# neka-nat/cupoch

Hardware: AMD Instinct MI355X
Metric: ICP iterations/sec (incl. kNN) on 10M-pt point-to-plane, 1/2/4/8 MI355X (higher is better)
Workload: dtype f32; 1 GPU; 10M-vs-10M point-to-plane ICP, radius 1-NN on an 8-ary kd-cell tree, r=2*N^(-1/3), uniform random clouds (BASELINE.md section 3); points=10000000, parallelism=single GPU, accumulate=f64

## Files before the change

cupoch_amd/_lib.py:

```python
import ctypes as C
import os
import shutil
import subprocess

_HERE = os.path.dirname(os.path.abspath(__file__))
ROOT = os.path.dirname(_HERE)
CSRC = os.path.join(_HERE, "csrc")
LIB_DIR = os.path.join(_HERE, "lib")
LIB_PATH = os.path.join(LIB_DIR, "libmi_icp.so")
INCLUDE = os.path.join(ROOT, "include")

HIPCC_FLAGS = ["--offload-arch=gfx950", "-O3", "-std=c++17", "-ffp-contract=off", "-fPIC", "-I/opt/rocm/include"]
UNITS = ["mi_icp", "mi_build", "mi_geometry", "mi_knn", "mi_comm", "mi_debug"]
OBJ_DIR = os.path.join(LIB_DIR, "obj")

MI_ICP_HOST, MI_ICP_DEVICE = 0, 1
EST_POINT_TO_POINT, EST_POINT_TO_PLANE, EST_SYMMETRIC, EST_GENERALIZED = 1, 2, 3, 5
EST_COLORED = 4


class MiIcpError(RuntimeError):
    pass


# ... 136 lines not shown
    "mi_icp_estimate_normals_knn": (_I, [_P, _P, _L, _I, _P, _I]),
    "mi_icp_estimate_normals_radius": (_I, [_P, _P, _L, _F, _I, _P, _I]),
    "mi_icp_search_knn": (_I, [_P, _P, _L, _I, _F, _P, _P, C.POINTER(_L), _I]),
    "mi_icp_set_target_colors": (_I, [_P, _P, _I]),
    "mi_icp_set_source_colors": (_I, [_P, _P, _I]),
    "mi_icp_set_lambda_geometric": (_I, [_P, _F]),
    "mi_icp_compute_color_gradients": (_I, [_P, _F, _I, _P, _I]),
    "mi_icp_registration_colored_icp": (_I, [_P, _F, _P, C.POINTER(Params), _F, C.POINTER(Result)]),
    "mi_icp_comm_unique_id": (_I, [_P]),
    "mi_icp_comm_init": (_I, [_P, _P, _I, _I]),
    "mi_icp_comm_init_local": (_I, [_P, C.c_char_p, _I, _I]),
    "mi_icp_comm_kind": (_I, [_P]),
    "mi_icp_comm_autotune": (_I, [_P, _I, _P, _P]),
    "mi_icp_comm_destroy": (_I, [_P]),
    "mi_icp_set_global_source_count": (_I, [_P, _L]),
    "mi_icp_spatial_order": (_I, [_P, _P, _L, _P, _I]),
    "mi_icp_set_iteration_callback": (_I, [_P, _P, _P]),
    "mi_icp_set_profiling": (_I, [_P, _I]),
    "mi_icp_get_profile": (_I, [_P, _P]),
    "mi_icp_debug_sort_pairs": (_I, [_P, _P, _P, _L, _I]),
    "mi_icp_debug_exclusive_scan": (_I, [_P, _P, _P, _L, _P]),
    "mi_icp_debug_morton_order": (_I, [_P, _P, _L, _P]),
    "mi_icp_debug_nn_stats": (_I, [_P, _P, _F, _I, _P]),
    "mi_icp_debug_nn_stats8": (_I, [_P, _P, _F, _I, _P]),
    "mi_icp_debug_get_tree": (_I, [_P, C.POINTER(_L), _P, _P]),
    "mi_icp_debug_drop_seeds": (_I, [_P]),
    "mi_icp_debug_last_search_kind": (_I, [_P]),
    "mi_icp_debug_last_voxel_path": (_I, [_P]),
    "mi_icp_debug_occupancy": (_I, [_I]),
    "mi_icp_debug_loop_counters": (_I, [_P, _P]),
    "mi_icp_debug_search_skip": (_I, [_P, _P, _P, _L, C.POINTER(_L), C.POINTER(_I)]),
    "mi_icp_debug_locate": (_I, [_P, _P, _P]),
    "mi_icp_debug_set_step_stamps": (_I, [_P, _I]),
    "mi_icp_debug_get_step_stamps": (_I, [_P, _P, C.POINTER(C.c_double)]),
    "mi_icp_debug_solve_both": (_I, [_I, _P, _I, C.c_float, _P, _P, _P, _P]),
    "mi_icp_debug_get_leaf_regions": (_I, [_P, _P]),
    "mi_icp_debug_get_leaf_halos": (_I, [_P, _P]),
    "mi_icp_debug_eigen3": (_I, [_I, _P, _L, _P, _P, _P]),
    "mi_icp_debug_odometry_image": (_I, [_P, _I, _I, _P, C.POINTER(_I), C.POINTER(_I)]),
}

_lib = None


def load():
    global _lib
    if _lib is not None:
        return _lib
    override = os.environ.get("MI_ICP_LIB_PATH")
    path = override or LIB_PATH
    if not os.path.exists(path):
        raise MiIcpError(
            "libmi_icp.so is not built (%s). Run `python -c 'import __graft_entry__ as g; "
            "g.build()'` or cupoch_amd._lib.build(); there is no CPU fallback." % LIB_PATH)
    try:
        lib = C.CDLL(path, mode=C.RTLD_GLOBAL)
    except OSError as e:
        raise MiIcpError("cannot load %s: %s" % (path, e))
    for name, (res, args) in SIGNATURES.items():
        if override and name.startswith("mi_icp_debug_") and not hasattr(lib, name):
            continue
        fn = getattr(lib, name)
        fn.restype = res
        fn.argtypes = args
    _lib = lib
    return lib
# ... 1 lines not shown
```

cupoch_amd/csrc/ctx.h:

```cpp
#pragma once
#include <hip/hip_runtime.h>
#include <rccl/rccl.h>

#include <algorithm>
#include <cmath>
#include <cstdarg>
#include <cstdio>
#include <cstdlib>
#include <cstring>
#include <string>

#include "../../include/mi_icp.h"
#include "../../include/mi_icp_debug.h"
#include "device_utils.h"
#include "host_solver.h"
#include "loop.h"
#include "mailbox.h"
#include "primitives.h"

namespace mi {
namespace eng {

using host::Mat4;

// ... 56 lines not shown

    mi::eng::DevBuf user_pairs;
    int64_t n_user_pairs = -1;

    mi::eng::DevBuf keys0, keys1, vals0, vals1, hist, scan_tmp, bounds_part, bounds;
    mi::eng::DevBuf partial, sys_dev, dense_idx, flags, pairs_out, seg_start;
    mi::eng::DevBuf stage[6];
    mi::eng::DevBuf tscale;
    mi::eng::DevBuf knn_idx, knn_flags;
    mi::eng::DevBuf dbs[4];
    mi::eng::DevBuf seg[4];
    float vx_refused_voxel = 0.0f;
    int64_t vx_refused_n = 0;
    int vx_order = 0;
    mi::eng::DevBuf vx_tab;
    mi::eng::DevBuf vpay[6];
    double* sys_host = nullptr;
    float* f_host = nullptr;
    uint32_t* u_host = nullptr;
    void* od_host = nullptr;
    int od_levels = 0, od_lw[MI_ICP_ODOMETRY_MAX_LEVELS] = {}, od_lh[MI_ICP_ODOMETRY_MAX_LEVELS] = {};
    const float* od_img[MI_ICP_ODOMETRY_MAX_LEVELS][8] = {};

    mi::eng::DevBuf loop_dev, ticket;
    mi::DevLoop* loop_host = nullptr;
    bool loop_active = false;
    mi_icp_iteration_fn iter_fn = nullptr;
    void* iter_user = nullptr;
    mi::eng::DevBuf loop_hist;
    float* hist_host = nullptr;
    int iter_reported = 0;
    float loop_r2 = 0.0f;
    int loop_est = 0;

    ncclComm_t comm = nullptr;
    int nranks = 1, rank = 0;
    mi::MailBox* mail_host = nullptr;
    mi::MailBox* mail_dev = nullptr;
    size_t mail_bytes = 0;
    std::string mail_name;
    bool mail_linked = false;
    unsigned long long* inbox = nullptr;
    unsigned long long* inbox_peer[mi::kMailRanks] = {};
    mi::eng::DevBuf inbox_table;
    bool comm_broken = false;
    int xchg = 0;
    uint32_t tune_epoch = 0;
    mi::eng::DevBuf mail_state;

    mi_icp_ctx* aux = nullptr;

    mi::eng::DevBuf stamps;
    bool stamps_on = false;
    bool profiling = false;
    static constexpr int kEvPairs = 16;
    hipEvent_t ev[4] = {nullptr, nullptr, nullptr, nullptr};
    hipEvent_t evp[2][kEvPairs][2] = {};
    int evp_n[2] = {0, 0};
    bool ev_pending_nn = false, ev_pending_red = false;
    double prof[8] = {0, 0, 0, 0, 0, 0, 0, 0};
};

namespace mi {
namespace eng {

inline float* lreg_of(const mi_icp_ctx* c) { return c->tblk.p ? (float*)c->tblk.p + mi::kLeafRegOffset : nullptr; }
// ... 72 lines not shown
        return MI_ICP_OK;
    }
    return ensure(c, stage, count, out);
}

template <class T>
int from_device(mi_icp_ctx* c, const T* dev, T* dst, size_t count, int mem_kind) {
    if (!dst || dst == dev || count == 0) return MI_ICP_OK;
    HIPCHK(c, hipMemcpyAsync(dst, dev, count * sizeof(T),
                             mem_kind == MI_ICP_DEVICE ? hipMemcpyDeviceToDevice
                                                       : hipMemcpyDeviceToHost,
                             c->stream));
    return MI_ICP_OK;
}

inline int drop_expiry(mi_icp_ctx* c) {
    c->skip_r2 = NAN;
    if (c->expiry_live && c->expiry.p) HIPCHK(c, hipMemsetAsync(c->expiry.p, 0xff, c->expiry.bytes, c->stream));
    c->expiry_live = false;
    return MI_ICP_OK;
}

inline uint32_t skip_live_shift(int64_t ns) {
    uint32_t shift = 0;
    while ((((ns + 63) / 64) >> (shift + 1)) >= 64) ++shift;
    return shift;
}
inline bool skip_pays(const mi_icp_ctx* c) {
    if (!c->loop_host || c->ns <= 0) return false;
    const int64_t samples = std::min<int64_t>(64, ((c->ns + 63) / 64) >> skip_live_shift(c->ns));
    int64_t held = 0;
    for (int64_t k = 0; k < samples; ++k) held += c->loop_host->live[k] ? 1 : 0;
    return samples > 0 && held * 4 >= samples;
}

inline int blocks_for(int64_t n, int per = 256) { return (int)std::max<int64_t>(1, (n + per - 1) / per); }

inline Xform make_xform(const Mat4& T) { return xform_from(T); }

inline Mat4 load_T(const float* T) {
    if (!T) return host::identity4();
    Mat4 m;
    std::memcpy(m.data(), T, sizeof(float) * 16);
    return m;
}

struct EvTimer {
    mi_icp_ctx* c;
    int slot;
    hipEvent_t stop = nullptr;
    bool pooled;
    EvTimer(mi_icp_ctx* ctx, int s, bool in_loop) : c(ctx), slot(s), pooled(in_loop) {
        if (!c->profiling) return;
        if (pooled) {
            if (c->evp_n[slot] >= mi_icp_ctx::kEvPairs) return;
            const int i = c->evp_n[slot]++;
            (void)hipEventRecord(c->evp[slot][i][0], c->stream);
            stop = c->evp[slot][i][1];
        } else {
            (void)hipEventRecord(c->ev[slot * 2], c->stream);
            stop = c->ev[slot * 2 + 1];
        }
    }
    ~EvTimer() {
        if (!stop) return;
        (void)hipEventRecord(stop, c->stream);
// ... 87 lines not shown
```

cupoch_amd/csrc/mi_debug.hip:

```cpp
#include "ctx.h"
#include <vector>
#include "halo_format.h"
#include "traverse.h"
#include "wave_solver.h"
#include "eigen3.h"

using namespace mi;
using namespace mi::eng;
using host::Mat4;

namespace mi {
__global__ __launch_bounds__(64) void solve_both_kernel(const double* systems, float det_thresh, float* out_serial,
                                                        float* out_wave, int32_t* ok_serial, int32_t* ok_wave) {
    __shared__ double s_sys[32];
    const int n = (int)blockIdx.x;
    if (threadIdx.x < 32) s_sys[threadIdx.x] = systems[(int64_t)n * 32 + threadIdx.x];
    __syncthreads();
    host::Mat4 W;
    const bool okw = wave_solve_system(s_sys, det_thresh, W);
    if (threadIdx.x < 16) out_wave[(int64_t)n * 16 + threadIdx.x] = select16(W.m, (int)threadIdx.x);
    if (threadIdx.x == 0) {
        ok_wave[n] = okw ? 1 : 0;
        host::Mat4 S;
        ok_serial[n] = host::solve_system(s_sys, det_thresh, S) ? 1 : 0;
// ... 116 lines not shown

int mi_icp_debug_solve_both(int device, const double* systems, int n, float det_thresh, float* out_serial,
                            float* out_wave, int32_t* ok_serial, int32_t* ok_wave) {
    if (!systems || n <= 0 || !out_serial || !out_wave || !ok_serial || !ok_wave) return MI_ICP_ERR_INVALID;
    if (hipSetDevice(device) != hipSuccess) return MI_ICP_ERR_NO_DEVICE;
    double* d_sys = nullptr;
    float* d_out = nullptr;
    int32_t* d_ok = nullptr;
    int rc = MI_ICP_ERR_HIP;
    if (hipMalloc(&d_sys, (size_t)n * 32 * sizeof(double)) == hipSuccess &&
        hipMalloc(&d_out, (size_t)n * 32 * sizeof(float)) == hipSuccess &&
        hipMalloc(&d_ok, (size_t)n * 2 * sizeof(int32_t)) == hipSuccess &&
        hipMemcpy(d_sys, systems, (size_t)n * 32 * sizeof(double), hipMemcpyHostToDevice) == hipSuccess) {
        mi::solve_both_kernel<<<n, 64>>>(d_sys, det_thresh, d_out, d_out + (size_t)n * 16, d_ok, d_ok + n);
        if (hipDeviceSynchronize() == hipSuccess &&
            hipMemcpy(out_serial, d_out, (size_t)n * 16 * sizeof(float), hipMemcpyDeviceToHost) == hipSuccess &&
            hipMemcpy(out_wave, d_out + (size_t)n * 16, (size_t)n * 16 * sizeof(float), hipMemcpyDeviceToHost) == hipSuccess &&
            hipMemcpy(ok_serial, d_ok, (size_t)n * sizeof(int32_t), hipMemcpyDeviceToHost) == hipSuccess &&
            hipMemcpy(ok_wave, d_ok + n, (size_t)n * sizeof(int32_t), hipMemcpyDeviceToHost) == hipSuccess)
            rc = MI_ICP_OK;
    }
    (void)hipFree(d_sys);
    (void)hipFree(d_out);
    (void)hipFree(d_ok);
    return rc;
}

int mi_icp_debug_set_step_stamps(mi_icp_ctx* c, int enable) {
    TRY(check_ctx(c));
    c->stamps_on = enable != 0;
    return MI_ICP_OK;
}

int mi_icp_debug_get_step_stamps(mi_icp_ctx* c, uint64_t* out32, double* ticks_per_us) {
    TRY(check_ctx(c));
    if (!out32 || !c->stamps.p) return fail(c, MI_ICP_ERR_STATE, "debug_get_step_stamps: no stamped loop has run on this context");
    HIPCHK(c, hipStreamSynchronize(c->stream));
    HIPCHK(c, hipMemcpy(out32, c->stamps.p, sizeof(uint64_t) * kStampWords, hipMemcpyDeviceToHost));
    if (ticks_per_us) {
        int khz = 0;
        *ticks_per_us = (hipDeviceGetAttribute(&khz, hipDeviceAttributeWallClockRate, c->device) == hipSuccess && khz > 0) ? khz / 1000.0 : 100.0;
    }
    return MI_ICP_OK;
}

int mi_icp_debug_loop_counters(mi_icp_ctx* c, int32_t* out4) {
    TRY(check_ctx(c));
    if (!out4 || !c->loop_host) return fail(c, MI_ICP_ERR_INVALID, "debug_loop_counters: bad arguments");
    HIPCHK(c, hipStreamSynchronize(c->stream));
    out4[0] = c->loop_host->iterations;
    out4[1] = c->loop_host->passes;
    out4[2] = c->loop_host->relocations;
    out4[3] = c->relocate_armed ? 1 : 0;
    return MI_ICP_OK;
}

int mi_icp_debug_drop_seeds(mi_icp_ctx* c) {
    TRY(check_ctx(c));
    c->nn_valid = false;
    return drop_expiry(c);
}

int mi_icp_debug_search_skip(mi_icp_ctx* c, double* state2, double* limits_out, int64_t capacity, int64_t* npackets, int* armed) {
    TRY(check_ctx(c));
    if (!state2 || !npackets || !armed || capacity < 0) return fail(c, MI_ICP_ERR_INVALID, "debug_search_skip: bad arguments");
    if (!c->loop_active || !c->loop_dev.p || !c->expiry.p || c->ns <= 0)
// ... 94 lines not shown
```

cupoch_amd/csrc/mi_icp.hip:

```cpp
#include "ctx.h"
#include "fused_small.h"
#include "lzf.h"
#include "nn_search.h"
#include "reduce.h"

using namespace mi;
using namespace mi::eng;
using host::Mat4;

namespace mi {

static __global__ __launch_bounds__(kStepThreads) void loop_step_kernel(DevLoop* st_g, double* sys_in, int resume, MailArgs mail) {
    __shared__ DevLoop st_s;
    loop_step_block(st_g, sys_in, resume, st_s, StepPre{false, 0u, 0.0, 0u}, mail);
}

namespace eng {

constexpr int64_t kPt2PlTwoFrom = (int64_t)4 << 20;

static int64_t coarse_first_min() {
    static const int64_t v = [] { const char* s = std::getenv("MI_ICP_COARSE_MIN"); return s ? std::atoll(s) : (int64_t)1 << 16; }();
    return v;
}
// ... 35 lines not shown
static decltype(&nn_packet_kernel<false, false>) nn_kernel(bool seeded, bool stats, bool stamp, bool gate) {
    if (gate) return stamp ? nn_packet_kernel<true, false, true, true> : nn_packet_kernel<true, false, false, true>;
    if (stats) return seeded ? nn_packet_kernel<true, true> : nn_packet_kernel<false, true>;
    if (seeded && stamp) return nn_packet_kernel<true, false, true>;
    return seeded ? nn_packet_kernel<true, false> : nn_packet_kernel<false, false>;
}

int launch_nn(mi_icp_ctx* c, const Mat4& T, float r2, bool seed, unsigned long long* stats, const DevLoop* loop) {
    if (c->ns <= 0) return MI_ICP_OK;
    int32_t* idx = (int32_t*)c->nn_idx.p;
    if (c->nt <= 0) {
        TRY(drop_expiry(c));
        fill_i32<<<blocks_for(c->ns), 256, 0, c->stream>>>(idx, c->ns, -1);
        KCHK(c);
        c->nn_valid = true;
        c->n_user_pairs = -1;
        return MI_ICP_OK;
    }
    const Xform X = make_xform(T);
    const bool use_seed = seed && c->nn_valid;
    bool have_halo;
    uint32_t* want = nullptr;
    if (loop) {
        TRY(loop_halo(c, &have_halo, &want));
    } else {
        if (use_seed) TRY(ensure_links(c));
        have_halo = halo_poll(c);
    }
    EvTimer t(c, 0, loop != nullptr);
    const bool self_seeded = !use_seed && !stats && c->ns >= coarse_first_min() && have_halo && planes_available(c);
    const bool limits = loop != nullptr && (use_seed || self_seeded) && !stats && c->expiry.p != nullptr;
    const bool may_skip = limits && use_seed && c->expiry_live && c->skip_r2 == r2;
    if (!may_skip) TRY(drop_expiry(c));
    const uint32_t run = (may_skip && skip_pays(c)) ? kSkipRun : 1u;
    if (self_seeded) TRY(launch_locate_by_planes(c, X, loop, 0));
    c->last_search_kind = use_seed ? 1 : (self_seeded ? 2 : 0);
    const PacketGrid g = packet_grid(c->ns, run);
    nn_kernel(use_seed || self_seeded, stats != nullptr, loop && c->stamps_on, run > 1u)<<<g.grid, kNNThreads, 0, c->stream>>>(
            (const float*)c->sx.p, (const float*)c->sy.p, (const float*)c->sz.p, (int)c->ns, (const float*)c->nodes.p,
            (const float*)c->tblk.p, (const float*)lreg_of(c), have_halo ? (const float*)c->thalo.p : nullptr, c->leaf_first,
            X, loop, r2, g.nblocks, idx, loop ? nullptr : (float*)c->nn_d2.p, stats, want,
            limits ? (double*)c->expiry.p : nullptr,
            limits ? reinterpret_cast<uint8_t*>(c->loop_dev.p) + offsetof(DevLoop, live) : nullptr, skip_live_shift(c->ns), run);
    KCHK(c);
    if (limits) {
        c->expiry_live = true;
        c->skip_r2 = r2;
    }
    c->nn_valid = true;
    c->n_user_pairs = -1;
    return MI_ICP_OK;
}

int occupancy_loop(int which) {
    int blocks = -1;
    hipError_t e = hipErrorInvalidValue;
    if (which == 1) e = hipOccupancyMaxActiveBlocksPerMultiprocessor(&blocks, nn_packet_kernel<true, false>, kNNThreads, 0);
    else if (which == 2) e = hipOccupancyMaxActiveBlocksPerMultiprocessor(&blocks, nn_packet_kernel<false, false>, kNNThreads, 0);
    else if (which == 3) e = hipOccupancyMaxActiveBlocksPerMultiprocessor(&blocks, reduce_pt2pl_kernel<2, 1>, kReduceThreads, 0);
    else return -1;
    return e == hipSuccess ? blocks : -2;
}

}
}

namespace {

int ensure_inverse_maps(mi_icp_ctx* c) {
    if (!c->inv_s_valid && c->ns > 0) {
        int32_t* inv;
        TRY(ensure(c, c->inv_s, (size_t)c->ns, &inv));
        invert_perm_source<<<blocks_for(c->ns), 256, 0, c->stream>>>((const int32_t*)c->sperm.p, (int)c->ns, inv);
        KCHK(c);
        c->inv_s_valid = true;
    }
// ... 56 lines not shown
        case kEstP2P: return reduce_kernel<kEstP2P, MODE>;
        case kEstPt2Pl: return reduce_kernel<kEstPt2Pl, MODE>;
        case kEstSym: return reduce_kernel<kEstSym, MODE>;
        case kEstColored: return reduce_kernel<kEstColored, MODE>;
        case kEstGICP: return reduce_kernel<kEstGICP, MODE>;
        default: return nullptr;
    }
}

int launch_reduce(mi_icp_ctx* c, int est, int mode, const Mat4& T, DevLoop* loop = nullptr, int step = 0) {
    double *partial, *sys;
    uint32_t* ticket;
    TRY(reduce_buffers(c, kReduceBlocks, &partial, &sys, &ticket));
    ReduceArgs a;
    a.sx = (const float*)c->sx.p;
    a.sy = (const float*)c->sy.p;
    a.sz = (const float*)c->sz.p;
    a.snrm = (const float4*)c->snrm.p;
    a.scov = (const float*)c->scov.p;
    a.tblk = (const float*)c->tblk.p;
    a.tnrm = (const float4*)c->tnrm.p;
    a.trec = c->t_has_rec ? (const float*)c->trec.p : nullptr;
    a.tcov = (const float*)c->tcov.p;
    a.tgrad = (const float4*)c->tgrad.p;
    a.sint = (const float*)c->sint.p;
    a.sqrt_lambda_geometric = std::sqrt(c->lambda_geometric);
    a.sqrt_lambda_photometric = std::sqrt(1.0f - c->lambda_geometric);
    a.nn_idx = (const int32_t*)c->nn_idx.p;
    a.pairs = nullptr;
    a.inv_s = a.inv_t = nullptr;
    a.ns = (int)c->ns;
    a.nt = (int)c->nt;
    a.count = c->ns;
    if (c->n_user_pairs >= 0) {
        TRY(ensure_inverse_maps(c));
        a.pairs = (const int32_t*)c->user_pairs.p;
        a.inv_s = (const int32_t*)c->inv_s.p;
        a.inv_t = (const int32_t*)c->inv_t.p;
        a.count = c->n_user_pairs;
    }
    if (c->ns <= 0 || c->nt <= 0 || (!a.pairs && !c->nn_valid)) a.count = 0;
    const int64_t wide = std::min<int64_t>(256, blocks_for(a.count, kReduceThreads));
    const int grid = (int)std::max<int64_t>(
            wide, std::min<int64_t>(kReduceBlocks, blocks_for(a.count, kReduceThreads * kReduceElemsPerThread)));
    const Xform X = make_xform(T);
    if (pt2pl_reduction(c, est, mode)) {
        const auto kernel = (a.count >= kPt2PlTwoFrom) ? pt2pl_kernel<2>(step, c->stamps_on) : pt2pl_kernel<4>(step, c->stamps_on);
        EvTimer t(c, 1, loop != nullptr);
        kernel<<<std::min(grid, 512), kReduceThreads, 0, c->stream>>>(a, X, loop, partial, ticket, sys,
                                                                     (step == 2) ? mail_args(c) : MailArgs{});
        KCHK(c);
        return MI_ICP_OK;
    }
    if (!estimator_ready(c, est)) {
        est = kEstP2P;
        mode = 1;
    }
    const auto kernel = mode ? generic_reduce_kernel<1>(est) : generic_reduce_kernel<0>(est);
    if (!kernel) return fail(c, MI_ICP_ERR_INVALID, "unknown estimation type %d", est);
    EvTimer t(c, 1, loop != nullptr);
    kernel<<<grid, kReduceThreads, 0, c->stream>>>(a, X, loop, partial, ticket, sys);
    KCHK(c);
    return MI_ICP_OK;
}

int fetch_system(mi_icp_ctx* c, double* out) {
    double* sys = (double*)c->sys_dev.p;
    TRY(allreduce_system(c));
    HIPCHK(c, hipMemcpyAsync(c->sys_host, sys, kSysSize * sizeof(double), hipMemcpyDeviceToHost, c->stream));
    const bool mail = mail_on(c);
    int32_t* err_host = reinterpret_cast<int32_t*>(c->sys_host + 40);
    if (mail) HIPCHK(c, hipMemcpyAsync(err_host, (const int32_t*)c->mail_state.p + 1, sizeof(int32_t), hipMemcpyDeviceToHost, c->stream));
    HIPCHK(c, hipStreamSynchronize(c->stream));
    collect_events(c);
    if (mail && *err_host) return comm_failed(c, "the ranks' exchange timed out (mailbox): a peer did not post its sums");
    std::memcpy(out, c->sys_host, kSysSize * sizeof(double));
    return MI_ICP_OK;
}

Mat4 solve_update(const mi_icp_ctx* c, int est, const double* sys, float det_thresh) {
// ... 371 lines not shown
    TRY(drop_expiry(c));
    const PacketGrid g = packet_grid(c->ns, kFusedPackets);
    double *partial, *sys;
    uint32_t* ticket;
    TRY(reduce_buffers(c, std::max<uint32_t>(kReduceBlocks, g.grid), &partial, &sys, &ticket));
    EvTimer t(c, 0, true);
    const auto kernel = (c->loop_est == kEstP2P) ? icp_small_iteration_kernel<kEstP2P> : icp_small_iteration_kernel<kEstPt2Pl>;
    kernel<<<g.grid, kReduceThreads, 0, c->stream>>>(
            (const float*)c->sx.p, (const float*)c->sy.p, (const float*)c->sz.p, (int)c->ns, (const float*)c->nodes.p,
            (const float*)c->tblk.p, (const float*)lreg_of(c), have_halo ? (const float*)c->thalo.p : nullptr, c->leaf_first,
            c->loop_r2, g.npackets, g.nblocks, (int32_t*)c->nn_idx.p, want, (const float*)c->trec.p, d, partial, ticket, sys);
    KCHK(c);
    c->last_search_kind = 1;
    return MI_ICP_OK;
}

static int step_in_reduction(const mi_icp_ctx* c) {
    if (!pt2pl_reduction(c, c->loop_est, 0)) return 0;
    if (mail_on(c)) return 2;
    return (!c->comm && !c->mail_dev) ? 1 : 0;
}

static int loop_enqueue_evaluation(mi_icp_ctx* c, bool seed) {
    DevLoop* d = (DevLoop*)c->loop_dev.p;
    if (seed && c->relocate_armed && c->halo_use && c->nn_valid && c->n_user_pairs < 0 && c->ns > 0 && c->nt > 0) {
        const Xform none = {};
        TRY(launch_locate_by_planes(c, none, d, 1));
    }
    if (fused_iteration_applies(c, seed)) return launch_fused_iteration(c, d);
    const Mat4 I = host::identity4();
    TRY(launch_nn(c, I, c->loop_r2, seed, nullptr, d));
    const int step = step_in_reduction(c);
    TRY(launch_reduce(c, c->loop_est, 0, I, d, step));
    if (step) return MI_ICP_OK;
    const bool mail = mail_on(c);
    if (!mail) TRY(allreduce_system(c));
    loop_step_kernel<<<1, kStepThreads, 0, c->stream>>>(d, (double*)c->sys_dev.p, 0, mail ? mail_args(c) : MailArgs{});
    KCHK(c);
    return MI_ICP_OK;
}

static bool halo_memory_free(const mi_icp_ctx* c) {
    size_t free_b = 0, total_b = 0;
    if (hipMemGetInfo(&free_b, &total_b) != hipSuccess) return false;
    return free_b >= (size_t)c->nts * 368u;
}

static int loop_run(mi_icp_ctx* c, int budget) {
    constexpr int kChunk = 8;
    constexpr int64_t kLarge = 500000, kHaloLongRun = 40, kHaloVeryLongRun = 1000;
    int chunk = kChunk;
    while (budget > 0) {
        const bool no_halo = !c->links_ready && !c->links_inflight && c->links_allowed && c->nt > 0;
        const bool undecided = no_halo && !c->halo_declined;
        if (c->links_inflight && !c->halo_declined) TRY(ensure_links(c));
        int n = (budget <= chunk + chunk / 2) ? budget : chunk;
        const bool grown = n == chunk;
        const bool several_ranks = c->comm != nullptr || c->mail_dev != nullptr;
        if (undecided && c->ns >= kLarge && !several_ranks) n = 1;
        const int passes_before = c->loop_host->passes;
        c->halo_use = halo_poll(c);
        const bool carried = c->relocate_armed && c->halo_use;
        const int relocations_before = c->loop_host->relocations;
        for (int i = 0; i < n; ++i) TRY(loop_enqueue_evaluation(c, true));
        const bool look = no_halo && (!c->halo_declined || (++c->halo_chunks & 7) == 0);
        if (look) HIPCHK(c, hipMemcpyAsync(c->u_host + 16, c->halo_want.p, kWantSlots * sizeof(uint32_t), hipMemcpyDeviceToHost, c->stream));
// ... 43 lines not shown
        return fail(c, MI_ICP_ERR_INVALID, "unknown estimation type %d", est);
    TRY(comm_usable(c));
    DevLoop& L = *c->loop_host;
    std::memset(&L, 0, sizeof(L));
    L.est = est;
    L.det_thresh = det_thresh;
    L.T = load_T(init);
    L.A = host::is_identity4(L.T) ? host::identity4() : L.T;
    L.X = xform_from(L.A);
    L.max_iterations = max_iterations;
    L.rel_fitness = rel_fitness;
    L.rel_rmse = rel_rmse;
    L.n_source_global = c->ns_global > 0 ? c->ns_global : c->ns;
    L.ready = estimator_ready(c, est) ? 1 : 0;
    L.history = 0ull;
    L.stamps = 0ull;
    L.travel = 0.0;
    L.fuzz = INFINITY;
    TRY(drop_expiry(c));
    const bool can_locate = planes_available(c) && c->ns >= coarse_first_min() && c->src_bounds.p != nullptr && c->nt > 0;
    L.near2_ptr = can_locate ? (uint64_t)(uintptr_t)((const float*)c->nodes.p + kRecordNear2) : 0ull;
    L.src_bounds_ptr = can_locate ? (uint64_t)(uintptr_t)c->src_bounds.p : 0ull;
    c->relocate_armed = c->relocate_possible = can_locate;
    if (c->stamps_on) {
        unsigned long long* st;
        TRY(ensure(c, c->stamps, kStampWords, &st));
        unsigned long long init[kStampWords] = {};
        init[0] = init[2] = ~0ull;
        HIPCHK(c, hipMemcpyAsync(st, init, sizeof(init), hipMemcpyHostToDevice, c->stream));
        HIPCHK(c, hipStreamSynchronize(c->stream));
        L.stamps = (uint64_t)(uintptr_t)st;
    }
    c->iter_reported = 0;
    if (c->iter_fn) {
        float* hist;
        TRY(ensure(c, c->loop_hist, (size_t)2 * kLoopHistory, &hist));
        if (!c->hist_host) HIPCHK(c, hipHostMalloc((void**)&c->hist_host, sizeof(float) * 2 * kLoopHistory, hipHostMallocDefault));
        L.history = (uint64_t)(uintptr_t)hist;
    }
    c->loop_active = false;
    c->loop_est = est;
    c->loop_r2 = max_distance * max_distance;
    if (max_distance <= 0.0f || (c->ns <= 0 && c->nranks <= 1)) {
        c->nn_valid = false;
        L.done = 1;
        return MI_ICP_OK;
    }
    DevLoop* d;
    TRY(ensure(c, c->loop_dev, 1, &d));
    HIPCHK(c, hipMemcpyAsync(d, &L, sizeof(DevLoop), hipMemcpyHostToDevice, c->stream));
    c->loop_active = true;
    c->halo_declined = false;
    c->halo_want_seen = 0;
    c->halo_looks = 0;
    c->halo_iters_unseen = 0;
    c->halo_chunks = 0;
    c->ran_loop = true;
    {
        uint32_t* want;
        TRY(ensure(c, c->halo_want, kWantSlots, &want));
        HIPCHK(c, hipMemsetAsync(want, 0, kWantSlots * sizeof(uint32_t), c->stream));
    }
    c->halo_use = halo_poll(c);
    if (c->halo_sticky && !c->halo_use) {
        if (c->links_inflight) {
            TRY(start_links_async(c));
// ... 66 lines not shown
```

cupoch_amd/csrc/nn_search.h:

```cpp
#pragma once
#include "device_utils.h"
#include "halo_format.h"
#include "kd_descend.h"
#include "loop.h"
#include "traverse.h"

namespace mi {

constexpr uint32_t kWantSlots = 1024u;
constexpr int kNNThreads = 64;
constexpr int kNNPacketsPerBlock = kNNThreads / 64;

constexpr int kItemQueue = 64 + 8 * 64;

struct PacketShared {
    unsigned long long best[64];
    uint32_t queue[kItemQueue];
};

__device__ __forceinline__ void eval_item(PacketShared& sh, const float* tblk_g, bool have, int ql, uint32_t L,
                                          float ox, float oy, float oz, float r2) {
    if (have) {
        const float4* line = reinterpret_cast<const float4*>(tblk_g + (size_t)L * kLeafFloats);
        const float4 x0 = line[0], x1 = line[1], y0 = line[2], y1 = line[3], z0 = line[4], z1 = line[5];
// ... 400 lines not shown
                const int32_t j = (int32_t)(L * (uint32_t)kLeaf + (uint32_t)w.k);
                if (w.m < best || (w.m == best && bidx >= 0 && j < bidx)) {
                    best = w.m;
                    bidx = j;
                }
            });
        }
    }

    if (valid) {
        if (!SEED || bidx != seed_j) nn_idx[i] = bidx;
        if (nn_d2) nn_d2[i] = (bidx >= 0) ? best : INFINITY;
    }
    if (STATS && lane == 0) {
        atomicAdd(stats + 0, (unsigned long long)steps);
        atomicAdd(stats + 1, (unsigned long long)batches);
        atomicAdd(stats + 2, 1ull);
        atomicMax(stats + 3, (unsigned long long)steps + (unsigned long long)batches);
        atomicAdd(stats + 4, (unsigned long long)halo_items);
        atomicAdd(stats + 5, halo_items ? 1ull : 0ull);
        atomicAdd(stats + 6, steps ? 1ull : 0ull);
        atomicAdd(stats + 7, (unsigned long long)walkers);
    }
    out.valid = valid;
    out.i = i;
    out.bidx = bidx;
    out.best = best;
    out.qx = qx;
    out.qy = qy;
    out.qz = qz;
    return true;
}

constexpr uint32_t kSkipRun = 8;
template <bool SEED, bool STATS, bool STAMP = false, bool GATE = false>
__global__ __launch_bounds__(kNNThreads) __attribute__((amdgpu_waves_per_eu(GATE ? 6 : (SEED ? 8 : 7), 8))) void nn_packet_kernel(
        const float* __restrict__ sx, const float* __restrict__ sy, const float* __restrict__ sz,
        int ns, const float* __restrict__ records_g, const float* __restrict__ tblk_g,
        const float* __restrict__ lreg_g, const float* __restrict__ halo_g, uint32_t leaf_first, Xform Tv, const DevLoop* __restrict__ loop, float r2, uint32_t nblocks, int32_t* __restrict__ nn_idx,
        float* __restrict__ nn_d2, unsigned long long* __restrict__ stats, uint32_t* __restrict__ want,
        double* __restrict__ expiry, uint8_t* __restrict__ live, uint32_t live_shift, uint32_t run) {
    __shared__ PacketShared s_pk[kNNPacketsPerBlock];
    uint32_t logical;
    if (!xcd_remap(nblocks, logical)) return;
    PacketResult unused;
    unsigned long long* stamps = (STAMP && loop) ? reinterpret_cast<unsigned long long*>(loop->stamps) : nullptr;
    if (STAMP && stamps && threadIdx.x == 0 && blockIdx.x < 64u) atomicMin(stamps + 0, stamp_now());
    if (!GATE) {
        (void)nn_packet_body<SEED, STATS>(s_pk[0], logical, sx, sy, sz, ns, records_g, tblk_g, lreg_g, halo_g, leaf_first, Tv, loop,
                                          r2, nn_idx, nn_d2, stats, want, unused, expiry, live, live_shift);
    } else {
        const uint32_t npackets = ((uint32_t)ns + 63u) >> 6, lane = (uint32_t)lane_id();
        const uint32_t first = logical * run;
        const bool mine = lane < run && first + lane < npackets;
        const double limit = expiry[mine ? first + lane : first];
        const double reach = loop->travel + loop->fuzz;
        uint32_t need = (loop->done != 0) ? 0u : (uint32_t)__ballot(mine && !(reach < limit));
        while (need != 0u) {
            const uint32_t k = (uint32_t)__builtin_ctz(need);
            need &= need - 1u;
            (void)nn_packet_body<true, false>(s_pk[0], first + k, sx, sy, sz, ns, records_g, tblk_g, lreg_g, halo_g, leaf_first, Xform{},
                                              loop, r2, nn_idx, nullptr, nullptr, want, unused, expiry, live, live_shift);
            __builtin_amdgcn_wave_barrier();
        }
    }
    if (STAMP && stamps && threadIdx.x == 0 && blockIdx.x + 256u >= gridDim.x) atomicMax(stamps + 1, stamp_now());
}

static __global__ __launch_bounds__(256) void locate_by_planes(
        const float* __restrict__ sx, const float* __restrict__ sy, const float* __restrict__ sz, int ns,
        const float2* __restrict__ cell_planes, int cell_levels, const uint32_t* __restrict__ gstart,
        const float2* __restrict__ gplanes, uint32_t nleaf, Xform Tv, const DevLoop* __restrict__ loop, int gated,
        int32_t* __restrict__ nn_idx, double* __restrict__ expiry) {
    Xform T = Tv;
    if (loop) {
        if (loop->done) return;
        if (gated && loop->relocate == 0) return;
        T = loop->X;
    }
    for (int64_t i = (int64_t)blockIdx.x * 256 + threadIdx.x; i < ns; i += (int64_t)gridDim.x * 256) {
        float qx, qy, qz;
        xform_point(T, sx[i], sy[i], sz[i], qx, qy, qz);
        const uint32_t cell = descend_cell(cell_planes, cell_levels, qx, qy, qz);
        const uint32_t g = gstart[cell];
        const uint32_t leaf = min(g * 512u + descend_group(gplanes + (size_t)g * 512u, qx, qy, qz), nleaf - 1u);
        nn_idx[i] = (int32_t)(leaf * (uint32_t)kLeaf);
        if (expiry != nullptr && (i & 63) == 0) expiry[i >> 6] = -(double)INFINITY;
    }
}


static __global__ __launch_bounds__(256) void export_dense(const int32_t* __restrict__ nn_idx,
                                                    const float* __restrict__ nn_d2,
                                                    const int32_t* __restrict__ sperm,
// ... 55 lines not shown
```

cupoch_amd/csrc/reduce.h:

```cpp
#pragma once
#include "device_utils.h"
#include "eigen3.h"
#include "loop.h"

namespace mi {

constexpr int kReduceThreads = 256;
constexpr int kReduceBlocks = 1024;

__device__ __forceinline__ void rotate_cov(const Xform& T, const float* C, M3& out) {
    const float R[3][3] = {{T.r00, T.r01, T.r02}, {T.r10, T.r11, T.r12}, {T.r20, T.r21, T.r22}};
    float RC[3][3];
#pragma unroll
    for (int c = 0; c < 3; ++c)
#pragma unroll
        for (int r = 0; r < 3; ++r)
            RC[r][c] = __builtin_fmaf(R[r][2], C[c * 3 + 2],
                                      __builtin_fmaf(R[r][1], C[c * 3 + 1], R[r][0] * C[c * 3 + 0]));
#pragma unroll
    for (int c = 0; c < 3; ++c)
#pragma unroll
        for (int r = 0; r < 3; ++r)
            out.m[r][c] = __builtin_fmaf(RC[r][2], R[c][2],
                                         __builtin_fmaf(RC[r][1], R[c][1], RC[r][0] * R[c][0]));
// ... 3 lines not shown
    int k = 0;
#pragma unroll
    for (int a = 0; a < 6; ++a)
#pragma unroll
        for (int b = a; b < 6; ++b, ++k) acc[k] = __builtin_fma((double)J[a], (double)J[b], acc[k]);
#pragma unroll
    for (int a = 0; a < 6; ++a) acc[21 + a] = __builtin_fma((double)J[a], (double)r, acc[21 + a]);
    acc[27] = __builtin_fma((double)r, (double)r, acc[27]);
}

struct __attribute__((packed, aligned(4))) F3 {
    float x, y, z;
};

struct ReduceArgs {
    const float* sx;
    const float* sy;
    const float* sz;
    const float4* snrm;
    const float* scov;
    const float* tblk;
    const float4* tnrm;
    const float* trec;
    const float4* tgrad;
    const float* sint;
    float sqrt_lambda_geometric, sqrt_lambda_photometric;
    const float* tcov;
    const int32_t* nn_idx;
    const int32_t* pairs;
    const int32_t* inv_s;
    const int32_t* inv_t;
    int ns, nt;
    int64_t count;
};

typedef double ReduceRows[kReduceThreads / 32][kSysSize];

__device__ __forceinline__ bool block_finish_rows(ReduceRows& red, double* __restrict__ partial,
                                                  uint32_t* __restrict__ ticket, double* __restrict__ out32,
                                                  StepPre* pre = nullptr, const DevLoop* pre_state = nullptr,
                                                  const uint32_t* pre_mail_seq = nullptr, unsigned long long* stamps = nullptr) {
    __shared__ uint32_t s_last;
    __syncthreads();
    if (threadIdx.x < 64) {
        if (threadIdx.x < kSysSize) {
            const int k = (int)threadIdx.x;
            __hip_atomic_store(&partial[(int64_t)blockIdx.x * kSysSize + k],
                               ((red[0][k] + red[1][k]) + red[2][k]) + red[3][k], __ATOMIC_RELAXED, __HIP_MEMORY_SCOPE_AGENT);
        }
        asm volatile("s_waitcnt vmcnt(0)" ::: "memory");
        if (threadIdx.x == 0) {
            const uint32_t t = __hip_atomic_fetch_add(ticket, 1u, __ATOMIC_RELAXED, __HIP_MEMORY_SCOPE_AGENT);
            const bool last = t == gridDim.x - 1u;
            if (last) __builtin_amdgcn_fence(__ATOMIC_ACQUIRE, "agent");
            if (last && stamps) stamps[3] = stamp_now();
            s_last = last ? 1u : 0u;
        }
    }
    __syncthreads();
    if (!s_last) return false;
    if (pre && pre_state) pre->word = loop_state_word(pre_state);
    if (pre && pre_mail_seq) pre->mail_seq = *pre_mail_seq;
    {
        const int k = (int)(threadIdx.x & 31u), part = (int)(threadIdx.x >> 5);
        constexpr int kParts = kReduceThreads / 32;
        const int nb = (int)gridDim.x;
// ... 289 lines not shown
            if (a.trec) {
                trec_gather(a.trec, j, vt, nt);
            } else {
                leaf_point(a.tblk, j, vt);
                const float4 n4 = a.tnrm[j];
                nt[0] = n4.x;
                nt[1] = n4.y;
                nt[2] = n4.z;
            }
            pt2pl_rows<MODE>(acc, vs, vt, nt);
        } else {
            leaf_point(a.tblk, j, vt);
            const float d[3] = {vs[0] - vt[0], vs[1] - vt[1], vs[2] - vt[2]};
            acc[28] += (double)sq3(d[0], d[1], d[2]);
            acc[29] += 1.0;
            if (EST == kEstSym) sym_rows<MODE>(acc, T, a, i, j, vs, vt, d);
            else if (EST == kEstColored) colored_rows<MODE>(acc, a, i, j, vs, vt, d);
            else if (EST == kEstGICP) gicp_rows<MODE>(acc, T, a, i, j, vs, d);
            else p2p_rows<MODE>(acc, vs, vt, d);
        }
    }

    block_finish(acc, partial, ticket, out32);
}

template <int kU, int STEP, bool STAMP = false>
__global__ __launch_bounds__(kReduceThreads) void reduce_pt2pl_kernel(ReduceArgs a, Xform Tv,
                                                                      DevLoop* __restrict__ loop,
                                                                      double* __restrict__ partial,
                                                                      uint32_t* __restrict__ ticket,
                                                                      double* __restrict__ out32, MailArgs mail) {
    const int64_t stride = (int64_t)gridDim.x * kReduceThreads;
    const int64_t k0 = (int64_t)blockIdx.x * kReduceThreads + threadIdx.x;
    int32_t j[kU];
    float px[kU], py[kU], pz[kU];
    auto fetch = [&](int64_t kb) {
#pragma unroll
        for (int u = 0; u < kU; ++u) {
            const int64_t k = kb + (int64_t)u * stride;
            const int64_t kc = (k < a.count) ? k : 0;
            j[u] = a.nn_idx[kc];
            px[u] = a.sx[kc];
            py[u] = a.sy[kc];
            pz[u] = a.sz[kc];
        }
    };
    fetch(k0);
    Xform T = Tv;
    unsigned long long* stamps = nullptr;
    if (loop) {
        if (loop->done) return;
        T = loop->X;
        if (STAMP) stamps = reinterpret_cast<unsigned long long*>(loop->stamps);
    }
    if (STAMP && stamps && threadIdx.x == 0) atomicMin(stamps + 2, stamp_now());
    double acc[30];
#pragma unroll
    for (int k = 0; k < 30; ++k) acc[k] = 0.0;
    for (int64_t kb = k0; kb < a.count; kb += stride * kU) {
        float vt[kU][3], nt[kU][3];
        bool have[kU];
#pragma unroll
        for (int u = 0; u < kU; ++u) {
            have[u] = (kb + (int64_t)u * stride) < a.count && j[u] >= 0;
            trec_gather(a.trec, have[u] ? j[u] : 0, vt[u], nt[u]);
        }
        float vs[kU][3];
#pragma unroll
        for (int u = 0; u < kU; ++u) xform_point(T, px[u], py[u], pz[u], vs[u][0], vs[u][1], vs[u][2]);
        fetch(kb + stride * kU);
#pragma unroll
        for (int u = 0; u < kU; ++u)
            if (have[u]) pt2pl_rows<0>(acc, vs[u], vt[u], nt[u]);
    }
    StepPre pre{STEP != 0, 0u, 0.0, 0u};
    const bool last = block_finish(acc, partial, ticket, out32, &pre, STEP ? loop : nullptr,
                                   (STEP == 2) ? mail.seq_dev : nullptr, STAMP ? stamps : nullptr);
    if (STEP && last) {
        __shared__ DevLoop st_s;
        if (STAMP && stamps && threadIdx.x == 0) stamps[4] = stamp_now();
        loop_step_block(loop, out32, 0, st_s, pre, (STEP == 2) ? mail : MailArgs{}, STAMP ? stamps : nullptr);
    }
}

}
```

cupoch_amd/engine.py:

```python
import ctypes as C

import numpy as np

from . import _lib
from ._lib import MI_ICP_DEVICE, MI_ICP_HOST, MiIcpError, Params, Result

try:
    import torch
except Exception:
    torch = None


def _is_tensor(a):
    return torch is not None and isinstance(a, torch.Tensor)


class _Buf:

    def __init__(self, a, dtype, cols, device_index, copy=False):
        self.keep = None
        self.ptr = None
        self.kind = MI_ICP_HOST
        self.device = None
        self.n = 0
# ... 606 lines not shown
        return out

    def comm_init(self, unique_id, nranks, rank):
        buf = C.create_string_buffer(bytes(unique_id), 128)
        self._chk(self._L.mi_icp_comm_init(self._ctx, buf, int(nranks), int(rank)))

    def comm_init_local(self, job_name, nranks, rank):
        self._chk(self._L.mi_icp_comm_init_local(self._ctx, str(job_name).encode(), int(nranks), int(rank)))

    def comm_kind(self):
        return int(self._L.mi_icp_comm_kind(self._ctx))

    def comm_autotune(self, exchanges=200):
        lat = (C.c_double * 3)()
        info = (C.c_int * 4)()
        self._chk(self._L.mi_icp_comm_autotune(self._ctx, int(exchanges), lat, info))
        names = ("host mailbox", "device inboxes", "rccl")
        show = lambda v: None if v == -1.0 else ("failed" if v < 0 else round(float(v), 3))
        return {"chosen": names[info[0] - 1] if 1 <= info[0] <= 3 else "none",
                "latency_us": {n: show(lat[i]) for i, n in enumerate(names)},
                "rccl_comm_count": int(info[1]), "exchanges": int(info[2]), "verified": bool(info[3])}

    def comm_destroy(self):
        self._chk(self._L.mi_icp_comm_destroy(self._ctx))

    def set_iteration_callback(self, fn):
        from ._lib import ITERATION_FN
        self._iter_cb = None if fn is None else ITERATION_FN(lambda _user, i, f, r: fn(int(i), float(f), float(r)))
        self._chk(self._L.mi_icp_set_iteration_callback(self._ctx, C.cast(self._iter_cb, C.c_void_p) if self._iter_cb else None, None))

    def set_step_stamps(self, enable=True):
        self._chk(self._L.mi_icp_debug_set_step_stamps(self._ctx, 1 if enable else 0))

    def get_step_stamps(self):
        out = np.zeros(32, np.uint64)
        tpu = C.c_double(0.0)
        self._chk(self._L.mi_icp_debug_get_step_stamps(self._ctx, out.ctypes.data_as(C.c_void_p), C.byref(tpu)))
        return out, float(tpu.value)

    def set_profiling(self, enable=True):
        self._chk(self._L.mi_icp_set_profiling(self._ctx, 1 if enable else 0))

    def get_profile(self):
        out = np.zeros(8, np.float64)
        self._chk(self._L.mi_icp_get_profile(self._ctx, out.ctypes.data_as(C.c_void_p)))
        return dict(nn_ms=out[0], nn_launches=int(out[1]), reduce_ms=out[2],
                    reduce_launches=int(out[3]), build_target_ms=out[4], build_source_ms=out[5],
                    halo_builds_by_loops=int(out[6]))


def comm_unique_id():
    L = _lib.load()
    buf = C.create_string_buffer(128)
    rc = L.mi_icp_comm_unique_id(buf)
    if rc != 0:
        raise MiIcpError("mi_icp_comm_unique_id failed (%d): RCCL not loadable" % rc)
    return bytes(buf.raw)


def _cov_in(covs):
    if covs is None:
        return None
    if _is_tensor(covs):
        c = covs.reshape(-1, 3, 3)
        return c.transpose(1, 2).contiguous().reshape(-1, 9)
    c = np.asarray(covs, np.float32).reshape(-1, 3, 3)
# ... 34 lines not shown
```

include/mi_icp_debug.h:

```cpp
#ifndef MI_ICP_DEBUG_H_
#define MI_ICP_DEBUG_H_
#include "mi_icp.h"
#ifdef __cplusplus
extern "C" {
#endif
MI_ICP_API int mi_icp_debug_sort_pairs(mi_icp_ctx* ctx, uint64_t* keys, uint32_t* vals,
                                       int64_t n, int key_bits);
MI_ICP_API int mi_icp_debug_exclusive_scan(mi_icp_ctx* ctx, const uint32_t* in, uint32_t* out,
                                           int64_t n, uint64_t* total);
MI_ICP_API int mi_icp_debug_morton_order(mi_icp_ctx* ctx, const float* xyz, int64_t n,
                                         uint32_t* order);
MI_ICP_API int mi_icp_debug_nn_stats(mi_icp_ctx* ctx, const float* T, float radius, int use_seed,
                                     uint64_t* out4);
MI_ICP_API int mi_icp_debug_nn_stats8(mi_icp_ctx* ctx, const float* T, float radius, int use_seed,
                                      uint64_t* out8);
MI_ICP_API int mi_icp_debug_drop_seeds(mi_icp_ctx* ctx);
MI_ICP_API int mi_icp_debug_last_search_kind(const mi_icp_ctx* ctx);
MI_ICP_API int mi_icp_debug_last_voxel_path(const mi_icp_ctx* ctx);
MI_ICP_API int mi_icp_debug_occupancy(int which);
MI_ICP_API int mi_icp_debug_loop_counters(mi_icp_ctx* ctx, int32_t* out4);
MI_ICP_API int mi_icp_debug_search_skip(mi_icp_ctx* ctx, double* state2, double* limits_out, int64_t capacity,
                                        int64_t* npackets, int* armed);
MI_ICP_API int mi_icp_debug_locate(mi_icp_ctx* ctx, const float* T, int32_t* leaf_out);
MI_ICP_API int mi_icp_debug_set_step_stamps(mi_icp_ctx* ctx, int enable);
MI_ICP_API int mi_icp_debug_get_step_stamps(mi_icp_ctx* ctx, uint64_t* out32, double* ticks_per_us);
MI_ICP_API int mi_icp_debug_solve_both(int device, const double* systems, int n, float det_thresh,
                                       float* out_serial, float* out_wave, int32_t* ok_serial, int32_t* ok_wave);
MI_ICP_API int mi_icp_debug_eigen3(int device, const float* A, int64_t n, float* eval, float* evec, float* S);
MI_ICP_API int mi_icp_debug_odometry_image(mi_icp_ctx* ctx, int level, int which, float* out, int* width, int* height);
MI_ICP_API int mi_icp_debug_get_tree(mi_icp_ctx* ctx, int64_t* info5, float* records_out,
                                     float* leaf_lines_out);
MI_ICP_API int mi_icp_debug_get_leaf_regions(mi_icp_ctx* ctx, float* regions_out);
MI_ICP_API int mi_icp_debug_get_leaf_halos(mi_icp_ctx* ctx, float* halos_out);
#ifdef __cplusplus
}
#endif
#endif
```

Before: 10170 iterations/s.

## Alternate reduction sweep direction and widen gated NN blocks to four waves

The point-to-plane reduction now walks its grid-stride loop backwards on every other loop iteration when the working set exceeds a 256 MiB on-die cache estimate. The intent is that data touched last by one sweep is still cached when the next sweep begins. Separately, the gated (skip) NN kernel now covers 64 packets per block using four waves: wave 0 ballots which packets need re-search and shares the mask through shared memory, and the needed packets are dealt round-robin across the waves. This adds a block barrier and more shared-memory packets per block, and it changes the load balance of the skip path. Debug hooks let the sweep mode be forced or inspected.

```diff
diff --git a/cupoch_amd/_lib.py b/cupoch_amd/_lib.py
--- a/cupoch_amd/_lib.py
+++ b/cupoch_amd/_lib.py
@@ -192,6 +192,8 @@
     "mi_icp_debug_search_skip": (_I, [_P, _P, _P, _L, C.POINTER(_L), C.POINTER(_I)]),
     "mi_icp_debug_locate": (_I, [_P, _P, _P]),
     "mi_icp_debug_set_step_stamps": (_I, [_P, _I]),
+    "mi_icp_debug_set_reduce_sweep": (_I, [_P, _I]),
+    "mi_icp_debug_get_reduce_sweep": (_I, [_P, C.POINTER(_L), C.POINTER(_I)]),
     "mi_icp_debug_get_step_stamps": (_I, [_P, _P, C.POINTER(C.c_double)]),
     "mi_icp_debug_solve_both": (_I, [_I, _P, _I, C.c_float, _P, _P, _P, _P]),
     "mi_icp_debug_get_leaf_regions": (_I, [_P, _P]),
diff --git a/cupoch_amd/csrc/ctx.h b/cupoch_amd/csrc/ctx.h
--- a/cupoch_amd/csrc/ctx.h
+++ b/cupoch_amd/csrc/ctx.h
@@ -112,6 +112,8 @@
     int iter_reported = 0;
     float loop_r2 = 0.0f;
     int loop_est = 0;
+    int64_t loop_reductions = 0;
+    int reduce_sweep_mode = 0;
 
     ncclComm_t comm = nullptr;
     int nranks = 1, rank = 0;
@@ -250,6 +252,14 @@
     int64_t held = 0;
     for (int64_t k = 0; k < samples; ++k) held += c->loop_host->live[k] ? 1 : 0;
     return samples > 0 && held * 4 >= samples;
+}
+
+constexpr int64_t kOnDieCacheBytes = (int64_t)256 << 20;
+inline bool reduce_sweep_reverse(const mi_icp_ctx* c, bool in_loop) {
+    if (c->reduce_sweep_mode == 1) return false;
+    if (c->reduce_sweep_mode == 2) return true;
+    const bool large = 16 * c->ns + 24 * c->nt > kOnDieCacheBytes;
+    return in_loop && (large || c->reduce_sweep_mode == 3) && (c->loop_reductions & 1) != 0;
 }
 
 inline int blocks_for(int64_t n, int per = 256) { return (int)std::max<int64_t>(1, (n + per - 1) / per); }
diff --git a/cupoch_amd/csrc/mi_debug.hip b/cupoch_amd/csrc/mi_debug.hip
--- a/cupoch_amd/csrc/mi_debug.hip
+++ b/cupoch_amd/csrc/mi_debug.hip
@@ -172,6 +172,21 @@
     return MI_ICP_OK;
 }
 
+int mi_icp_debug_set_reduce_sweep(mi_icp_ctx* c, int mode) {
+    TRY(check_ctx(c));
+    if (mode < 0 || mode > 3) return fail(c, MI_ICP_ERR_INVALID, "debug_set_reduce_sweep: mode %d is not one of 0..3", mode);
+    c->reduce_sweep_mode = mode;
+    return MI_ICP_OK;
+}
+
+int mi_icp_debug_get_reduce_sweep(mi_icp_ctx* c, int64_t* enqueued, int* next_reverse) {
+    TRY(check_ctx(c));
+    if (!enqueued || !next_reverse) return fail(c, MI_ICP_ERR_INVALID, "debug_get_reduce_sweep: bad arguments");
+    *enqueued = c->loop_reductions;
+    *next_reverse = reduce_sweep_reverse(c, true) ? 1 : 0;
+    return MI_ICP_OK;
+}
+
 int mi_icp_debug_get_step_stamps(mi_icp_ctx* c, uint64_t* out32, double* ticks_per_us) {
     TRY(check_ctx(c));
     if (!out32 || !c->stamps.p) return fail(c, MI_ICP_ERR_STATE, "debug_get_step_stamps: no stamped loop has run on this context");
diff --git a/cupoch_amd/csrc/mi_icp.hip b/cupoch_amd/csrc/mi_icp.hip
--- a/cupoch_amd/csrc/mi_icp.hip
+++ b/cupoch_amd/csrc/mi_icp.hip
@@ -91,16 +91,16 @@
     const bool limits = loop != nullptr && (use_seed || self_seeded) && !stats && c->expiry.p != nullptr;
     const bool may_skip = limits && use_seed && c->expiry_live && c->skip_r2 == r2;
     if (!may_skip) TRY(drop_expiry(c));
-    const uint32_t run = (may_skip && skip_pays(c)) ? kSkipRun : 1u;
+    const bool gate = may_skip && skip_pays(c);
     if (self_seeded) TRY(launch_locate_by_planes(c, X, loop, 0));
     c->last_search_kind = use_seed ? 1 : (self_seeded ? 2 : 0);
-    const PacketGrid g = packet_grid(c->ns, run);
-    nn_kernel(use_seed || self_seeded, stats != nullptr, loop && c->stamps_on, run > 1u)<<<g.grid, kNNThreads, 0, c->stream>>>(
+    const PacketGrid g = packet_grid(c->ns, gate ? kGateRun : 1u);
+    nn_kernel(use_seed || self_seeded, stats != nullptr, loop && c->stamps_on, gate)<<<g.grid, gate ? kGateThreads : kNNThreads, 0, c->stream>>>(
             (const float*)c->sx.p, (const float*)c->sy.p, (const float*)c->sz.p, (int)c->ns, (const float*)c->nodes.p,
             (const float*)c->tblk.p, (const float*)lreg_of(c), have_halo ? (const float*)c->thalo.p : nullptr, c->leaf_first,
             X, loop, r2, g.nblocks, idx, loop ? nullptr : (float*)c->nn_d2.p, stats, want,
             limits ? (double*)c->expiry.p : nullptr,
-            limits ? reinterpret_cast<uint8_t*>(c->loop_dev.p) + offsetof(DevLoop, live) : nullptr, skip_live_shift(c->ns), run);
+            limits ? reinterpret_cast<uint8_t*>(c->loop_dev.p) + offsetof(DevLoop, live) : nullptr, skip_live_shift(c->ns));
     KCHK(c);
     if (limits) {
         c->expiry_live = true;
@@ -223,6 +223,7 @@
     a.ns = (int)c->ns;
     a.nt = (int)c->nt;
     a.count = c->ns;
+    a.reverse = 0;
     if (c->n_user_pairs >= 0) {
         TRY(ensure_inverse_maps(c));
         a.pairs = (const int32_t*)c->user_pairs.p;
@@ -237,6 +238,7 @@
     const Xform X = make_xform(T);
     if (pt2pl_reduction(c, est, mode)) {
         const auto kernel = (a.count >= kPt2PlTwoFrom) ? pt2pl_kernel<2>(step, c->stamps_on) : pt2pl_kernel<4>(step, c->stamps_on);
+        a.reverse = reduce_sweep_reverse(c, loop != nullptr) ? 1 : 0;
         EvTimer t(c, 1, loop != nullptr);
         kernel<<<std::min(grid, 512), kReduceThreads, 0, c->stream>>>(a, X, loop, partial, ticket, sys,
                                                                      (step == 2) ? mail_args(c) : MailArgs{});
@@ -674,6 +676,7 @@
     TRY(launch_nn(c, I, c->loop_r2, seed, nullptr, d));
     const int step = step_in_reduction(c);
     TRY(launch_reduce(c, c->loop_est, 0, I, d, step));
+    ++c->loop_reductions;
     if (step) return MI_ICP_OK;
     const bool mail = mail_on(c);
     if (!mail) TRY(allreduce_system(c));
@@ -783,6 +786,7 @@
         L.stamps = (uint64_t)(uintptr_t)st;
     }
     c->iter_reported = 0;
+    c->loop_reductions = 0;
     if (c->iter_fn) {
         float* hist;
         TRY(ensure(c, c->loop_hist, (size_t)2 * kLoopHistory, &hist));
diff --git a/cupoch_amd/csrc/nn_search.h b/cupoch_amd/csrc/nn_search.h
--- a/cupoch_amd/csrc/nn_search.h
+++ b/cupoch_amd/csrc/nn_search.h
@@ -456,15 +456,17 @@
     return true;
 }
 
-constexpr uint32_t kSkipRun = 8;
+constexpr uint32_t kGateRun = 64;
+constexpr int kGateWaves = 4;
+constexpr int kGateThreads = 64 * kGateWaves;
 template <bool SEED, bool STATS, bool STAMP = false, bool GATE = false>
-__global__ __launch_bounds__(kNNThreads) __attribute__((amdgpu_waves_per_eu(GATE ? 6 : (SEED ? 8 : 7), 8))) void nn_packet_kernel(
+__global__ __launch_bounds__(GATE ? kGateThreads : kNNThreads) __attribute__((amdgpu_waves_per_eu(GATE ? 6 : (SEED ? 8 : 7), 8))) void nn_packet_kernel(
         const float* __restrict__ sx, const float* __restrict__ sy, const float* __restrict__ sz,
         int ns, const float* __restrict__ records_g, const float* __restrict__ tblk_g,
         const float* __restrict__ lreg_g, const float* __restrict__ halo_g, uint32_t leaf_first, Xform Tv, const DevLoop* __restrict__ loop, float r2, uint32_t nblocks, int32_t* __restrict__ nn_idx,
         float* __restrict__ nn_d2, unsigned long long* __restrict__ stats, uint32_t* __restrict__ want,
-        double* __restrict__ expiry, uint8_t* __restrict__ live, uint32_t live_shift, uint32_t run) {
-    __shared__ PacketShared s_pk[kNNPacketsPerBlock];
+        double* __restrict__ expiry, uint8_t* __restrict__ live, uint32_t live_shift) {
+    __shared__ PacketShared s_pk[GATE ? kGateWaves : kNNPacketsPerBlock];
     uint32_t logical;
     if (!xcd_remap(nblocks, logical)) return;
     PacketResult unused;
@@ -474,16 +476,26 @@
         (void)nn_packet_body<SEED, STATS>(s_pk[0], logical, sx, sy, sz, ns, records_g, tblk_g, lreg_g, halo_g, leaf_first, Tv, loop,
                                           r2, nn_idx, nn_d2, stats, want, unused, expiry, live, live_shift);
     } else {
+        __shared__ unsigned long long s_need;
         const uint32_t npackets = ((uint32_t)ns + 63u) >> 6, lane = (uint32_t)lane_id();
-        const uint32_t first = logical * run;
-        const bool mine = lane < run && first + lane < npackets;
-        const double limit = expiry[mine ? first + lane : first];
-        const double reach = loop->travel + loop->fuzz;
-        uint32_t need = (loop->done != 0) ? 0u : (uint32_t)__ballot(mine && !(reach < limit));
-        while (need != 0u) {
-            const uint32_t k = (uint32_t)__builtin_ctz(need);
-            need &= need - 1u;
-            (void)nn_packet_body<true, false>(s_pk[0], first + k, sx, sy, sz, ns, records_g, tblk_g, lreg_g, halo_g, leaf_first, Xform{},
+        const uint32_t wave = (uint32_t)__builtin_amdgcn_readfirstlane((int)(threadIdx.x >> 6));
+        const uint32_t first = logical * kGateRun;
+        if (wave == 0u) {
+            const bool mine = first + lane < npackets;
+            const double limit = expiry[mine ? first + lane : first];
+            const double reach = loop->travel + loop->fuzz;
+            const unsigned long long all = (loop->done != 0) ? 0ull : __ballot(mine && !(reach < limit));
+            if (lane == 0u) s_need = all;
+        }
+        __syncthreads();
+        const unsigned long long held = s_need;
+        unsigned long long need = ((unsigned long long)(uint32_t)__builtin_amdgcn_readfirstlane((int)(uint32_t)(held >> 32)) << 32) |
+                                  (unsigned long long)(uint32_t)__builtin_amdgcn_readfirstlane((int)(uint32_t)held);
+        for (uint32_t rank = 0u; need != 0ull; ++rank) {
+            const uint32_t k = (uint32_t)__builtin_ctzll(need);
+            need &= need - 1ull;
+            if ((rank & (uint32_t)(kGateWaves - 1)) != wave) continue;
+            (void)nn_packet_body<true, false>(s_pk[wave], first + k, sx, sy, sz, ns, records_g, tblk_g, lreg_g, halo_g, leaf_first, Xform{},
                                               loop, r2, nn_idx, nullptr, nullptr, want, unused, expiry, live, live_shift);
             __builtin_amdgcn_wave_barrier();
         }
diff --git a/cupoch_amd/csrc/reduce.h b/cupoch_amd/csrc/reduce.h
--- a/cupoch_amd/csrc/reduce.h
+++ b/cupoch_amd/csrc/reduce.h
@@ -59,6 +59,7 @@
     const int32_t* inv_t;
     int ns, nt;
     int64_t count;
+    int reverse;
 };
 
 typedef double ReduceRows[kReduceThreads / 32][kSysSize];
@@ -414,20 +415,27 @@
                                                                       double* __restrict__ out32, MailArgs mail) {
     const int64_t stride = (int64_t)gridDim.x * kReduceThreads;
     const int64_t k0 = (int64_t)blockIdx.x * kReduceThreads + threadIdx.x;
+    const uint32_t span = (uint32_t)stride * (uint32_t)kU;
+    int64_t kb = k0, hop = (int64_t)span;
+    if (a.reverse) {
+        const uint32_t nb = (k0 < a.count) ? ((uint32_t)(a.count - k0 - 1) / span + 1u) : 0u;
+        kb = k0 + ((int64_t)nb - 1) * (int64_t)span;
+        hop = -(int64_t)span;
+    }
     int32_t j[kU];
     float px[kU], py[kU], pz[kU];
-    auto fetch = [&](int64_t kb) {
+    auto fetch = [&](int64_t from) {
 #pragma unroll
         for (int u = 0; u < kU; ++u) {
-            const int64_t k = kb + (int64_t)u * stride;
-            const int64_t kc = (k < a.count) ? k : 0;
+            const int64_t k = from + (int64_t)u * stride;
+            const int64_t kc = ((uint64_t)k < (uint64_t)a.count) ? k : 0;
             j[u] = a.nn_idx[kc];
             px[u] = a.sx[kc];
             py[u] = a.sy[kc];
             pz[u] = a.sz[kc];
         }
     };
-    fetch(k0);
+    fetch(kb);
     Xform T = Tv;
     unsigned long long* stamps = nullptr;
     if (loop) {
@@ -439,7 +447,7 @@
     double acc[30];
 #pragma unroll
     for (int k = 0; k < 30; ++k) acc[k] = 0.0;
-    for (int64_t kb = k0; kb < a.count; kb += stride * kU) {
+    for (; (uint64_t)kb < (uint64_t)a.count; kb += hop) {
         float vt[kU][3], nt[kU][3];
         bool have[kU];
 #pragma unroll
@@ -450,7 +458,7 @@
         float vs[kU][3];
 #pragma unroll
         for (int u = 0; u < kU; ++u) xform_point(T, px[u], py[u], pz[u], vs[u][0], vs[u][1], vs[u][2]);
-        fetch(kb + stride * kU);
+        fetch(kb + hop);
 #pragma unroll
         for (int u = 0; u < kU; ++u)
             if (have[u]) pt2pl_rows<0>(acc, vs[u], vt[u], nt[u]);
diff --git a/cupoch_amd/engine.py b/cupoch_amd/engine.py
--- a/cupoch_amd/engine.py
+++ b/cupoch_amd/engine.py
@@ -662,6 +662,14 @@
     def set_step_stamps(self, enable=True):
         self._chk(self._L.mi_icp_debug_set_step_stamps(self._ctx, 1 if enable else 0))
 
+    def set_reduce_sweep(self, mode):
+        self._chk(self._L.mi_icp_debug_set_reduce_sweep(self._ctx, int(mode)))
+
+    def get_reduce_sweep(self):
+        n, rev = C.c_int64(0), C.c_int(0)
+        self._chk(self._L.mi_icp_debug_get_reduce_sweep(self._ctx, C.byref(n), C.byref(rev)))
+        return int(n.value), bool(rev.value)
+
     def get_step_stamps(self):
         out = np.zeros(32, np.uint64)
         tpu = C.c_double(0.0)
diff --git a/include/mi_icp_debug.h b/include/mi_icp_debug.h
--- a/include/mi_icp_debug.h
+++ b/include/mi_icp_debug.h
@@ -23,6 +23,8 @@
                                         int64_t* npackets, int* armed);
 MI_ICP_API int mi_icp_debug_locate(mi_icp_ctx* ctx, const float* T, int32_t* leaf_out);
 MI_ICP_API int mi_icp_debug_set_step_stamps(mi_icp_ctx* ctx, int enable);
+MI_ICP_API int mi_icp_debug_set_reduce_sweep(mi_icp_ctx* ctx, int mode);
+MI_ICP_API int mi_icp_debug_get_reduce_sweep(mi_icp_ctx* ctx, int64_t* enqueued, int* next_reverse);
 MI_ICP_API int mi_icp_debug_get_step_stamps(mi_icp_ctx* ctx, uint64_t* out32, double* ticks_per_us);
 MI_ICP_API int mi_icp_debug_solve_both(int device, const double* systems, int n, float det_thresh,
                                        float* out_serial, float* out_wave, int32_t* ok_serial, int32_t* ok_wave);
```

Measured after the change: 10910 iterations/s, median of 6. +7.2%, better.
